# ru1ven/KeypointFusion

Measured on NVIDIA B200. Metric: fusion-path RGB-D samples/sec, higher is better.
Workload: dtype bf16

## Files before the change

keypointfusion_b200/csrc/token_stack.cu:

```cuda
#include "tcgen05.cuh"

namespace kpf {

constexpr int TS_C = 128;
constexpr int TS_WORKERS = 512;
constexpr int TS_NT = TS_WORKERS + 32;
constexpr int TS_RING = 4;
constexpr int TS_SLOT = 2048;
constexpr int TS_MAXG = 64;
constexpr int TS_VEC = 10 * TS_C;
constexpr int TS_PLANE = 512;
constexpr uint32_t ACC_Q = 0, ACC_K = 32, ACC_V = 64, ACC_X = 96, ACC_F = 128, ACC_S = 256, ACC_O = 384;
constexpr uint32_t VT_HI = 128, VT_LO = 144;

struct TokParams {
    const float* x;
    const float* y;
    const float* r3d;
    const float* desa;
    const float* jf;
    const uint4* wmat;
    const int4* wseq;
    const float* wvec;
    float* tokens_out;
    float* pred_out;
    float* out_cj;
    float* out_jc;
    int out_jc_stride, out_jc_c0;
    int B, J, D, L, F, pre, cross, Fc, G, fmt;
    const unsigned long long* peer_bases;
    const int* xstep;
    int world, row0, rows_total;
};

constexpr int XCHG_HEADER_FLOATS = 16;

__device__ __forceinline__ float gelu_erf(float x) {
    const float z = fabsf(x) * 0.70710678118654752f;
    const float t = __fdividef(1.f, 1.f + 0.3275911f * z);
    const float poly = ((((1.061405429f * t - 1.453152027f) * t + 1.421413741f) * t - 0.284496736f) * t + 0.254829592f) * t;
    const float erf_abs = 1.f - poly * __expf(-z * z);
    return 0.5f * x * (1.f + copysignf(erf_abs, x));
}

template <int NV>
__device__ __forceinline__ void warp_reduce_scatter(float* v, int lane) {
    int off = 16;
#pragma unroll
    for (int n = NV; n > 1; n >>= 1, off >>= 1) {
        const bool upper = (lane & off) != 0;
#pragma unroll
        for (int i = 0; i < n / 2; ++i) {
            const float send = upper ? v[i] : v[i + n / 2];
            const float recv = __shfl_xor_sync(0xffffffffu, send, off);
            v[i] = (upper ? v[i + n / 2] : v[i]) + recv;
        }
    }
#pragma unroll
    for (; off > 0; off >>= 1) v[0] += __shfl_xor_sync(0xffffffffu, v[0], off);
}

template <int FMT>
__global__ void __launch_bounds__(TS_NT, 1) token_stack_kernel(const TokParams p) {
    extern __shared__ __align__(128) unsigned char ts_smem[];
    uint4* wslot = reinterpret_cast<uint4*>(ts_smem);
    uint4* bufX = wslot + TS_RING * TS_SLOT;
    uint4* bufY = bufX + 2 * TS_PLANE;
    uint4* bufQ = bufY + 2 * TS_PLANE;
    uint4* bufK = bufQ + 2 * TS_PLANE;
    uint4* bufAt = bufK + 2 * TS_PLANE;
    float* sVec = reinterpret_cast<float*>(bufAt + 128);
    float* sRed = sVec + 2 * TS_VEC;
    float* sSum = sRed + 512;
    float* sHead = sSum + 512;
    float* sLead = sHead + 1024;
    __shared__ __align__(8) uint64_t full[TS_RING], empty[TS_RING], vec_full[2], vec_empty[2], bars[4];
    __shared__ uint32_t tmem_slot;

    const int tid = threadIdx.x, lane = tid & 31, w = tid >> 5, q = w & 3, c = (w >> 2) & 3;
    const int f = 32 * q + lane;
    const int J = p.J, C = TS_C, G = p.G;
    constexpr int fmt = FMT;
    const int b = blockIdx.x;
    const int warp_u = warp_index_uniform();
    const bool producer = warp_u == TS_WORKERS / 32;

    pdl_launch_dependents();
    if (warp_u == 0) tmem_alloc(&tmem_slot, 512);
    if (tid == 32) {
        for (int i = 0; i < TS_RING; ++i) {
            mbar_init(&full[i], 1);
            mbar_init(&empty[i], 1);
        }
        for (int i = 0; i < 2; ++i) {
            mbar_init(&vec_full[i], 1);
            mbar_init(&vec_empty[i], 1);
        }
        for (int i = 0; i < 4; ++i) mbar_init(&bars[i], 1);
        fence_mbar_init();
    }
    tc_fence_before();
    __syncthreads();
    tc_fence_after();
    const uint32_t tmem0 = tmem_slot;
    const uint32_t tmem = tmem0 + ((uint32_t)(32 * q) << 16);

    const int D = p.D, shift = p.L > 0 ? D - C : 0;
    const float* vp = p.wvec;
    const float *qpos = nullptr, *kpos = nullptr, *cross_vec = nullptr, *bfu = nullptr, *pos = nullptr, *bemb = nullptr,
                *Wres_lead = nullptr, *Wres_feat = nullptr, *bres = nullptr, *Wcls = nullptr, *bcls = nullptr, *enc_vec = nullptr;
    if (p.cross) {
        qpos = vp;
        kpos = qpos + J * C;
        cross_vec = kpos + J * C;
        vp = cross_vec + TS_VEC;
    }
    if (p.pre) {
        bfu = vp;
        vp += C;
    }
    if (p.L > 0) {
        pos = vp;
        bemb = pos + J * C;
        Wres_lead = bemb + C;
        Wres_feat = Wres_lead + 48;
        bres = Wres_feat + 3 * C;
        Wcls = bres + 4;
        bcls = Wcls + 3 * C;
        enc_vec = bcls + 4;
    }
    const int n_layers = (p.cross ? 1 : 0) + p.L;
    auto layer_vec = [&](int it) { return (p.cross && it == 0) ? cross_vec : enc_vec + (size_t)(it - (p.cross ? 1 : 0)) * TS_VEC; };

    if (producer) {
        if (elect_one()) {
            for (int e = 0; e < G; ++e) {
                const int4 s = __ldg(p.wseq + e);
                if (s.z >= 0) {
                    const int it = s.z;
                    if (it >= 2) mbar_wait(&vec_empty[it & 1], ((it >> 1) - 1) & 1);
                    mbar_expect_tx(&vec_full[it & 1], TS_VEC * 4);
                    tma_bulk_g2s(sVec + (it & 1) * TS_VEC, layer_vec(it), TS_VEC * 4, &vec_full[it & 1]);
                }
                const int slot = e & (TS_RING - 1);
                if (e >= TS_RING) mbar_wait(&empty[slot], ((e >> 2) - 1) & 1);
                mbar_expect_tx(&full[slot], (uint32_t)s.y * 16);
                tma_bulk_g2s(wslot + slot * TS_SLOT, p.wmat + s.x, (uint32_t)s.y * 16, &full[slot]);
            }
        }
        __syncwarp();
        pdl_wait();
        return;
    }

    auto wsync = [&]() { named_bar_sync(1, 512); };
    uint32_t bar_phase[4] = {0, 0, 0, 0};
    auto wait_bar = [&](int i) {
        mbar_wait(&bars[i], bar_phase[i]);
        bar_phase[i] ^= 1;
        tc_fence_after();
    };
    auto sync_for_mma = [&]() {
        fence_proxy_async();
        tc_fence_before();
        wsync();
    };
    int g = 0;
    auto slot_addr = [&](int e) { return smem_u32(wslot + (e & (TS_RING - 1)) * TS_SLOT); };
    auto wait_full = [&](int e) { mbar_wait(&full[e & (TS_RING - 1)], (e >> 2) & 1); };
    auto issue_proj = [&](uint32_t acc, const uint4* act, int e, bool accumulate) {
        const uint32_t id = umma_idesc_f16(128, 32, false, true, fmt, fmt);
#pragma unroll 1
        for (int h = 0; h < 2; ++h) {
            wait_full(e + h);
            tc_fence_after();
            SmemOp a, bo;
            a.hi = slot_addr(e + h); a.lo = a.hi + 16384; a.lbo = 2048; a.sbo = 128;
            bo.hi = smem_u32(act) + h * 4096; bo.lo = bo.hi + TS_PLANE * 16; bo.lbo = 512; bo.sbo = 128;
            umma_gemm3_ss<64>(tmem0 + acc, a, bo, id, accumulate || h > 0);
            umma_commit(&empty[(e + h) & (TS_RING - 1)]);
        }
    };
    const uint32_t xidx = (uint32_t)((f >> 3) * 32 + c * 8 + (f & 7));
    auto write_act = [&](uint4* buf, const float* v) {
        uint4 hi, lo;
        split8<FMT>(v, hi, lo);
        buf[xidx] = hi;
        buf[TS_PLANE + xidx] = lo;
    };
    bool tokv[8];
#pragma unroll
    for (int i = 0; i < 8; ++i) tokv[i] = 8 * c + i < J;
    auto load_tok = [&](const float* base, int ld, float* v) {
#pragma unroll
        for (int i = 0; i < 8; ++i) v[i] = tokv[i] ? __ldg(base + (size_t)(8 * c + i) * ld + f) : 0.f;
    };
    auto head_partial = [&](int part, const float* v, const float* W) {
        float hx[32];
        const float w0 = __ldg(W + f), w1 = __ldg(W + C + f), w2 = __ldg(W + 2 * C + f);
#pragma unroll
        for (int i = 0; i < 8; ++i) {
            hx[3 * i] = v[i] * w0;
            hx[3 * i + 1] = v[i] * w1;
            hx[3 * i + 2] = v[i] * w2;
        }
#pragma unroll
        for (int i = 24; i < 32; ++i) hx[i] = 0.f;
        warp_reduce_scatter<32>(hx, lane);
        sHead[((part * 4 + q) * 4 + c) * 32 + lane] = hx[0];
    };

    if (tid < 128) sLead[tid] = 0.f;
    wsync();
    pdl_wait();
    float resid[8] = {0.f, 0.f, 0.f, 0.f, 0.f, 0.f, 0.f, 0.f};
    const float qscale = rsqrtf((float)(C / 4));
    int red_par = 0;

    if (p.cross) {
        float a[8], e[8];
        load_tok(p.x + (size_t)b * J * C, C, a);
        load_tok(qpos, C, e);
#pragma unroll
        for (int i = 0; i < 8; ++i) {
            resid[i] = a[i];
            e[i] += a[i];
        }
        write_act(bufX, e);
        load_tok(p.y + (size_t)b * J * C, C, a);
        load_tok(kpos, C, e);
#pragma unroll
        for (int i = 0; i < 8; ++i) e[i] += a[i];
        write_act(bufY, e);
    }

    auto fusion_prologue = [&](float* a) {
        float v[8];
        const float* dsrc = p.desa + (size_t)b * 3 * J * C;
        load_tok(dsrc, C, v);
        write_act(bufX, v);
        load_tok(dsrc + (size_t)J * C, C, v);
        write_act(bufY, v);
        load_tok(dsrc + (size_t)2 * J * C, C, v);
        write_act(bufQ, v);
        load_tok(p.jf + (size_t)b * J * C, C, v);
        write_act(bufK, v);
        sync_for_mma();
        if (warp_u == 0) {
            tc_fence_after();
            if (elect_one()) {
                issue_proj(ACC_X, bufX, g, false);
                issue_proj(ACC_X, bufY, g + 2, true);
                issue_proj(ACC_X, bufQ, g + 4, true);
                issue_proj(ACC_X, bufK, g + 6, true);
                umma_commit(&bars[0]);
            }
            __syncwarp();
        }
        g += 8;
        const float bb = __ldg(bfu + f);
        wait_bar(0);
        tmem_ld<8>(tmem + ACC_X + 8 * c, a);
#pragma unroll
        for (int i = 0; i < 8; ++i) a[i] = tokv[i] ? fmaxf(a[i] + bb, 0.f) : 0.f;
    };
    float pre_a[8] = {0.f, 0.f, 0.f, 0.f, 0.f, 0.f, 0.f, 0.f};
    if (p.pre) {
        fusion_prologue(pre_a);
        if (p.L == 0 && p.tokens_out) {
#pragma unroll
            for (int i = 0; i < 8; ++i)
                if (tokv[i]) p.tokens_out[((size_t)b * J + 8 * c + i) * C + f] = pre_a[i];
        }
    }

    for (int it = 0; it < n_layers; ++it) {
        const bool is_cross = p.cross && it == 0;
        if (it == (p.cross ? 1 : 0) && p.L > 0) {
            if (p.pre) {
                head_partial(0, pre_a, Wres_feat);
                write_act(bufX, pre_a);
            }
            if (!p.pre && !p.cross) {
                float v[8];
                load_tok(p.x + (size_t)b * J * D + shift, D, v);
                head_partial(0, v, Wres_feat);
                write_act(bufX, v);
            }
            if (p.cross) head_partial(0, resid, Wres_feat);
            if (shift > 0 && w == 0) {
                const int t = lane;
                const float* lead = p.cross ? p.r3d + ((size_t)b * J + t) * shift : p.x + ((size_t)b * J + t) * D;
                float tl[16];
#pragma unroll
                for (int i = 0; i < 16; ++i) tl[i] = (t < J && i < shift) ? __ldg(lead + i) : 0.f;
#pragma unroll
                for (int k = 0; k < 3; ++k) {
                    float s = 0.f;
#pragma unroll
                    for (int i = 0; i < 16; ++i) s += tl[i] * __ldg(Wres_lead + 16 * k + i);
                    sLead[4 * t + k] = s;
                }
                uint4 hi, lo;
                split8<FMT>(tl, hi, lo);
                bufAt[t] = hi;
                bufAt[64 + t] = lo;
                split8<FMT>(tl + 8, hi, lo);
                bufAt[32 + t] = hi;
                bufAt[96 + t] = lo;
            }
            sync_for_mma();
            if (warp_u == 0) {
                tc_fence_after();
                if (elect_one()) {
                    issue_proj(ACC_X, bufX, g, false);
                    if (shift > 0) {
                        wait_full(g + 2);
                        tc_fence_after();
                        SmemOp a, bo;
                        a.hi = slot_addr(g + 2); a.lo = a.hi + 256 * 16; a.lbo = 2048; a.sbo = 128;
                        bo.hi = smem_u32(bufAt); bo.lo = bo.hi + 64 * 16; bo.lbo = 512; bo.sbo = 128;
                        umma_gemm3_ss<16>(tmem0 + ACC_X, a, bo, umma_idesc_f16(128, 32, false, false, fmt, fmt), true);
                        umma_commit(&empty[(g + 2) & (TS_RING - 1)]);
                    }
                    umma_commit(&bars[0]);
                }
                __syncwarp();
            }
            g += shift > 0 ? 3 : 2;
            float e[8];
            load_tok(pos, C, e);
            const float bb = __ldg(bemb + f);
            wait_bar(0);
            float a[8];
            tmem_ld<8>(tmem + ACC_X + 8 * c, a);
#pragma unroll
            for (int i = 0; i < 8; ++i) resid[i] = a[i] = tokv[i] ? a[i] + bb + e[i] : 0.f;
            write_act(bufX, a);
        }

        const float* sv = sVec + (it & 1) * TS_VEC;
        const uint4* kv_src = is_cross ? bufY : bufX;
        const int F = is_cross ? p.Fc : p.F;
        const int act = is_cross ? 0 : 1;
        const float eps = is_cross ? 1e-5f : 1e-12f;

        sync_for_mma();
        if (warp_u == 0) {
            tc_fence_after();
            if (elect_one()) {
                if (it >= 1) mbar_arrive(&vec_empty[(it - 1) & 1]);
                issue_proj(ACC_K, kv_src, g, false);
                umma_commit(&bars[1]);
                issue_proj(ACC_Q, bufX, g + 2, false);
                umma_commit(&bars[0]);
            }
            __syncwarp();
        }
        mbar_wait(&vec_full[it & 1], (it >> 1) & 1);
        const float bq = sv[f], bk = sv[C + f], bv = sv[2 * C + f], bo_ = sv[3 * C + f], g1 = sv[4 * C + f], be1 = sv[5 * C + f],
                    b2 = sv[7 * C + f], g2 = sv[8 * C + f], be2 = sv[9 * C + f];
        const float* b1 = sv + 6 * C;
        const uint32_t qidx = (uint32_t)((lane >> 3) * 128 + (4 * q + c) * 8 + (lane & 7));
        wait_bar(1);
        {
            float a[8];
            tmem_ld<8>(tmem + ACC_K + 8 * c, a);
#pragma unroll
            for (int i = 0; i < 8; ++i) a[i] = tokv[i] ? a[i] + bk : 0.f;
            uint4 hi, lo;
            split8<FMT>(a, hi, lo);
            bufK[qidx] = hi;
            bufK[TS_PLANE + qidx] = lo;
        }
        wait_bar(0);
        {
            float a[8];
            tmem_ld<8>(tmem + ACC_Q + 8 * c, a);
#pragma unroll
            for (int i = 0; i < 8; ++i) a[i] = tokv[i] ? (a[i] + bq) * qscale : 0.f;
            uint4 hi, lo;
            split8<FMT>(a, hi, lo);
            bufQ[qidx] = hi;
            bufQ[TS_PLANE + qidx] = lo;
        }
        sync_for_mma();
        if (warp_u == 0) {
            tc_fence_after();
            if (elect_one()) {
                SmemOp a, bo;
                a.hi = smem_u32(bufQ); a.lo = a.hi + TS_PLANE * 16; a.lbo = 2048; a.sbo = 128;
                bo.hi = smem_u32(bufK); bo.lo = bo.hi + TS_PLANE * 16; bo.lbo = 2048; bo.sbo = 128;
                umma_gemm3_ss<32>(tmem0 + ACC_S, a, bo, umma_idesc_f16(128, 128, true, true, fmt, fmt), false);
                umma_commit(&bars[0]);
                issue_proj(ACC_V, kv_src, g + 4, false);
                umma_commit(&bars[1]);
            }
            __syncwarp();
        }
        wait_bar(0);
        {
            float sa[32], own[8];
            tmem_ld_nw<32>(tmem + ACC_S + 32 * q, sa);
            tmem_ld_nw<8>(tmem + ACC_S + 32 * q + 8 * c, own);
            tmem_wait_ld();
            float mx = -INFINITY;
#pragma unroll
            for (int i = 0; i < 32; ++i) mx = fmaxf(mx, i < J ? sa[i] : -INFINITY);
            float psum = 0.f;
            const bool qv = lane < J;
#pragma unroll
            for (int i = 0; i < 8; ++i) {
                own[i] = (qv && tokv[i]) ? __expf(own[i] - mx) : 0.f;
                psum += own[i];
            }
            sSum[c * 128 + f] = psum;
            uint4 hi, lo;
            split8<FMT>(own, hi, lo);
            bufQ[c * 128 + f] = hi;
            bufQ[TS_PLANE + c * 128 + f] = lo;
        }
        wait_bar(1);
        {
            float a[8];
            tmem_ld<8>(tmem + ACC_V + 8 * c, a);
#pragma unroll
            for (int i = 0; i < 8; ++i) a[i] = tokv[i] ? a[i] + bv : 0.f;
            uint4 hi, lo;
            split8<FMT>(a, hi, lo);
            tmem_st_nw<4>(tmem + VT_HI + 4 * c, reinterpret_cast<const float*>(&hi));
            tmem_st_nw<4>(tmem + VT_LO + 4 * c, reinterpret_cast<const float*>(&lo));
            tmem_wait_st();
        }
        sync_for_mma();
        if (warp_u == 0) {
            tc_fence_after();
            if (elect_one()) {
                TmemOp a;
                a.hi = tmem0 + VT_HI; a.lo = tmem0 + VT_LO;
                SmemOp bo;
                bo.hi = smem_u32(bufQ); bo.lo = bo.hi + TS_PLANE * 16; bo.lbo = 2048; bo.sbo = 128;
                umma_gemm3_ts<32>(tmem0 + ACC_O, a, bo, umma_idesc_f16(128, 128, false, false, fmt, fmt), false);
                umma_commit(&bars[0]);
            }
            __syncwarp();
        }
        float inv[8];
        {
            float s8[8] = {0.f, 0.f, 0.f, 0.f, 0.f, 0.f, 0.f, 0.f};
#pragma unroll
            for (int k = 0; k < 4; ++k) {
                const float4 u0 = *reinterpret_cast<const float4*>(sSum + k * 128 + 32 * q + 8 * c);
                const float4 u1 = *reinterpret_cast<const float4*>(sSum + k * 128 + 32 * q + 8 * c + 4);
                s8[0] += u0.x; s8[1] += u0.y; s8[2] += u0.z; s8[3] += u0.w;
                s8[4] += u1.x; s8[5] += u1.y; s8[6] += u1.z; s8[7] += u1.w;
            }
#pragma unroll
            for (int i = 0; i < 8; ++i) inv[i] = tokv[i] ? 1.f / s8[i] : 0.f;
        }
        wait_bar(0);
        {
            float a[8];
            tmem_ld<8>(tmem + ACC_O + 32 * q + 8 * c, a);
#pragma unroll
            for (int i = 0; i < 8; ++i) a[i] *= inv[i];
            write_act(bufX, a);
        }
        auto resid_ln = [&](float bias, float gam, float bet) {
            float v[16];
            tmem_ld<8>(tmem + ACC_X + 8 * c, v);
#pragma unroll
            for (int i = 0; i < 8; ++i) {
                v[i] += bias + resid[i];
                resid[i] = v[i];
                v[8 + i] = v[i] * v[i];
            }
            warp_reduce_scatter<16>(v, lane);
            float* red = sRed + red_par * 256;
            red_par ^= 1;
            if ((lane & 1) == 0) red[(c * 4 + q) * 16 + (lane >> 1)] = v[0];
            wsync();
            float st[16];
#pragma unroll
            for (int i = 0; i < 16; ++i) st[i] = 0.f;
#pragma unroll
            for (int k = 0; k < 4; ++k) {
#pragma unroll
                for (int j4 = 0; j4 < 4; ++j4) {
                    const float4 u = *reinterpret_cast<const float4*>(red + (c * 4 + k) * 16 + 4 * j4);
                    st[4 * j4] += u.x; st[4 * j4 + 1] += u.y; st[4 * j4 + 2] += u.z; st[4 * j4 + 3] += u.w;
                }
            }
            float y[8];
#pragma unroll
            for (int i = 0; i < 8; ++i) {
                const float mean = st[i] * (1.f / C);
                const float rstd = rsqrtf(fmaxf(st[8 + i] * (1.f / C) - mean * mean, 0.f) + eps);
                resid[i] = y[i] = tokv[i] ? (resid[i] - mean) * rstd * gam + bet : 0.f;
            }
            write_act(bufX, y);
        };
        sync_for_mma();
        if (warp_u == 0) {
            tc_fence_after();
            if (elect_one()) {
                issue_proj(ACC_X, bufX, g + 6, false);
                umma_commit(&bars[0]);
            }
            __syncwarp();
        }
        wait_bar(0);
        resid_ln(bo_, g1, be1);
        const int nffn = F == 16 ? 1 : 4;
        sync_for_mma();
        if (warp_u == 0) {
            tc_fence_after();
            if (elect_one()) {
                SmemOp a, bo;
                a.hi = smem_u32(bufX); a.lo = a.hi + TS_PLANE * 16; a.lbo = 512; a.sbo = 128;
                if (F == 16) {
                    wait_full(g + 8);
                    tc_fence_after();
                    bo.hi = slot_addr(g + 8); bo.lo = bo.hi + 256 * 16; bo.lbo = 256; bo.sbo = 128;
                    umma_gemm3_ss<128>(tmem0 + ACC_F, a, bo, umma_idesc_f16(128, 16, true, false, fmt, fmt), false);
                } else {
#pragma unroll 1
                    for (int h = 0; h < 2; ++h) {
                        wait_full(g + 8 + h);
                        tc_fence_after();
                        SmemOp ah = a;
                        ah.hi += h * 4096; ah.lo += h * 4096;
                        bo.hi = slot_addr(g + 8 + h); bo.lo = bo.hi + 16384; bo.lbo = 2048; bo.sbo = 128;
                        umma_gemm3_ss<64>(tmem0 + ACC_F, ah, bo, umma_idesc_f16(128, 128, true, false, fmt, fmt), h > 0);
                        umma_commit(&empty[(g + 8 + h) & (TS_RING - 1)]);
                    }
                }
                umma_commit(&bars[0]);
            }
            __syncwarp();
        }
        wait_bar(0);
        if (q == 0) {
            const bool tv = lane < J;
            if (F == 16) {
                float a[4];
                tmem_ld<4>(tmem0 + ACC_F + 4 * c, a);
#pragma unroll
                for (int i = 0; i < 4; ++i) {
                    const float u = a[i] + b1[4 * c + i];
                    a[i] = tv ? (act == 1 ? gelu_erf(u) : fmaxf(u, 0.f)) : 0.f;
                }
                uint2 hi, lo;
                split2<FMT>(a[0], a[1], hi.x, lo.x);
                split2<FMT>(a[2], a[3], hi.y, lo.y);
                reinterpret_cast<uint2*>(bufY + (c >> 1) * 32 + lane)[c & 1] = hi;
                reinterpret_cast<uint2*>(bufY + TS_PLANE + (c >> 1) * 32 + lane)[c & 1] = lo;
            } else {
#pragma unroll 1
                for (int j4 = 0; j4 < 4; ++j4) {
                    float a[8];
                    tmem_ld<8>(tmem0 + ACC_F + 32 * c + 8 * j4, a);
#pragma unroll
                    for (int i = 0; i < 8; ++i) {
                        const float u = a[i] + b1[32 * c + 8 * j4 + i];
                        a[i] = tv ? (act == 1 ? gelu_erf(u) : fmaxf(u, 0.f)) : 0.f;
                    }
                    uint4 hi, lo;
                    split8<FMT>(a, hi, lo);
                    bufY[(4 * c + j4) * 32 + lane] = hi;
                    bufY[TS_PLANE + (4 * c + j4) * 32 + lane] = lo;
                }
            }
        }
        sync_for_mma();
        if (warp_u == 0) {
            tc_fence_after();
            if (elect_one()) {
                SmemOp a, bo;
                bo.hi = smem_u32(bufY); bo.lo = bo.hi + TS_PLANE * 16; bo.lbo = 512; bo.sbo = 128;
                const uint32_t id = umma_idesc_f16(128, 32, false, false, fmt, fmt);
                if (F == 16) {
                    a.hi = slot_addr(g + 8) + 512 * 16; a.lo = a.hi + 256 * 16; a.lbo = 2048; a.sbo = 128;
                    umma_gemm3_ss<16>(tmem0 + ACC_X, a, bo, id, false);
                    umma_commit(&empty[(g + 8) & (TS_RING - 1)]);
                } else {
#pragma unroll 1
                    for (int h = 0; h < 2; ++h) {
                        wait_full(g + 10 + h);
                        tc_fence_after();
                        a.hi = slot_addr(g + 10 + h); a.lo = a.hi + 16384; a.lbo = 2048; a.sbo = 128;
                        SmemOp bh = bo;
                        bh.hi += h * 4096; bh.lo += h * 4096;
                        umma_gemm3_ss<64>(tmem0 + ACC_X, a, bh, id, h > 0);
                        umma_commit(&empty[(g + 10 + h) & (TS_RING - 1)]);
                    }
                }
                umma_commit(&bars[0]);
            }
            __syncwarp();
        }
        wait_bar(0);
        resid_ln(b2, g2, be2);
        g += 8 + nffn;
    }

    if (p.cross && p.L == 0) {
#pragma unroll
        for (int i = 0; i < 8; ++i) {
            const int t = 8 * c + i;
            if (tokv[i]) {
                if (p.out_cj) p.out_cj[((size_t)b * C + f) * J + t] = resid[i];
                if (p.out_jc) p.out_jc[((size_t)b * J + t) * p.out_jc_stride + p.out_jc_c0 + f] = resid[i];
            }
        }
    }
    if (p.L > 0) {
        head_partial(1, resid, Wcls);
        if (p.tokens_out) {
#pragma unroll
            for (int i = 0; i < 8; ++i)
                if (tokv[i]) p.tokens_out[((size_t)b * J + 8 * c + i) * C + f] = resid[i];
        }
        wsync();
        if (tid < 96 && p.pred_out) {
            const int t = tid / 3, k = tid - 3 * t, cc = t >> 3, i = t & 7;
            if (t < J) {
                float o = __ldg(bres + k) + __ldg(bcls + k) + sLead[4 * t + k];
#pragma unroll
                for (int part = 0; part < 2; ++part)
#pragma unroll
                    for (int qq = 0; qq < 4; ++qq) o += sHead[((part * 4 + qq) * 4 + cc) * 32 + 3 * i + k];
                p.pred_out[((size_t)b * J + t) * 3 + k] = o;
                if (p.peer_bases) {
                    const size_t off = XCHG_HEADER_FLOATS + ((size_t)(*p.xstep & 1) * p.rows_total + p.row0 + b) * J * 3 + (size_t)t * 3 + k;
                    for (int r = 0; r < p.world; ++r) reinterpret_cast<float*>(p.peer_bases[r])[off] = o;
                }
            }
        }
        if (p.peer_bases && tid < 96) {
            __threadfence_system();
            named_bar_sync(2, 96);
            if (tid < p.world) asm volatile("red.relaxed.sys.global.add.u32 [%0], 1;" ::"l"(p.peer_bases[tid]) : "memory");
        }
    }
    tc_fence_before();
    wsync();
    if (warp_u == 0) tmem_dealloc(tmem0, 512);
}

constexpr size_t TS_SMEM = (size_t)(TS_RING * TS_SLOT + 8 * TS_PLANE + 128) * 16 + (size_t)(2 * TS_VEC + 512 + 512 + 1024 + 128) * 4;

}

__global__ void exchange_wait_kernel(const unsigned int* arrived, int* xstep, unsigned int per_step, int* inflight, int mode) {
    if (*inflight) {
        const unsigned int expected = ((unsigned int)*xstep + 1u) * per_step;
        const long long t0 = clock64();
        while (true) {
            unsigned int v;
            asm volatile("ld.acquire.sys.global.u32 %0, [%1];" : "=r"(v) : "l"(arrived) : "memory");
            if ((int)(v - expected) >= 0) break;
            if (clock64() - t0 > 8000000000ll) __trap();
        }
        *xstep = *xstep + 1;
    }
    *inflight = mode == 0 ? 1 : 0;
}

extern "C" int kpf_exchange_wait(const void* exchange_buffer, int* xstep, int samples_per_step, int* inflight, int mode, cudaStream_t stream) {
    KPF_REQUIRE(exchange_buffer != nullptr && xstep != nullptr && inflight != nullptr && samples_per_step >= 1 && (mode == 0 || mode == 1));
    exchange_wait_kernel<<<1, 1, 0, stream>>>((const unsigned int*)exchange_buffer, xstep, (unsigned int)samples_per_step, inflight, mode);
    KPF_CHECK_LAUNCH();
    return 0;
}

extern "C" int kpf_token_stack(const float* x, const float* y, const float* r3d, const float* desa, const float* jf, const void* wmat,
                               const void* wseq, const float* wvec, int n_weights, int cross, int pre, int B, int J, int D, int L, int F,
                               int Fc, int fmt, float* tokens_out, float* pred_out, float* out_cj, float* out_jc, int out_jc_stride,
                               int out_jc_c0, const void* peer_bases, const int* xstep, int world, int row0, int rows_total,
                               cudaStream_t stream) {
    using namespace kpf;
    KPF_REQUIRE(B >= 0 && J >= 1 && J <= 32 && L >= 0 && (cross || pre || L > 0));
    KPF_REQUIRE(fmt == FMT_F16 || fmt == FMT_BF16);
    if (B == 0) return 0;
    KPF_REQUIRE(L == 0 || F == 16 || F == 128);
    KPF_REQUIRE(!cross || (y != nullptr && (Fc == 16 || Fc == 128)));
    KPF_REQUIRE(L == 0 || D == TS_C || (D > TS_C && D <= TS_C + 16));
    KPF_REQUIRE(!pre || (desa != nullptr && jf != nullptr && !cross && (L == 0 || D == TS_C)));
    KPF_REQUIRE(!(cross && L > 0) || (r3d != nullptr && D > TS_C));
    KPF_REQUIRE(n_weights <= TS_MAXG);
    const int per_cross = 8 + (Fc == 16 ? 1 : 4), per_layer = 8 + (F == 16 ? 1 : 4);
    KPF_REQUIRE(n_weights == (cross ? per_cross : 0) + (pre ? 8 : 0) + (L > 0 ? 2 + (D > TS_C ? 1 : 0) + per_layer * L : 0));
    KPF_REQUIRE(((uintptr_t)wmat % 16) == 0 && ((uintptr_t)wseq % 16) == 0);
    TokParams p;
    p.x = x; p.y = y; p.r3d = r3d; p.desa = desa; p.jf = jf; p.wmat = (const uint4*)wmat; p.wseq = (const int4*)wseq; p.wvec = wvec;
    p.tokens_out = tokens_out; p.pred_out = pred_out; p.out_cj = out_cj; p.out_jc = out_jc; p.out_jc_stride = out_jc_stride;
    p.out_jc_c0 = out_jc_c0; p.B = B; p.J = J; p.D = D; p.L = L; p.F = F; p.pre = pre; p.cross = cross; p.Fc = Fc; p.G = n_weights; p.fmt = fmt;
    KPF_REQUIRE(peer_bases == nullptr || (xstep != nullptr && world >= 1 && row0 >= 0 && row0 + B <= rows_total && L > 0));
    p.peer_bases = (const unsigned long long*)peer_bases; p.xstep = xstep; p.world = world; p.row0 = row0; p.rows_total = rows_total;
    auto kern = fmt == FMT_F16 ? token_stack_kernel<FMT_F16> : token_stack_kernel<FMT_BF16>;
    cudaError_t e = kpf::set_smem(kern, TS_SMEM);
    if (e != cudaSuccess) return (int)e;
    e = kpf::launch_pdl(kern, dim3(B), dim3(TS_NT), TS_SMEM, stream, p);
    if (e != cudaSuccess) return (int)e;
    KPF_CHECK_LAUNCH();
    return 0;
}
```

Baseline: 138,300.

## Process two batch samples per CTA with N=64 UMMA tiles

Each CTA now handles two samples, doubling the MMA N dimension from 32 to 64 so every weight tile streamed through the TMA ring is reused across two samples, and the grid is halved. Activation buffers, TMEM accumulator columns and reduction scratch are resized, the weight ring shrinks from 4 to 3 slots to fit shared memory, and the Y buffer is folded into K/Q buffers with the fusion prologue split into two MMA phases. This reduces weight traffic per sample but halves the CTA count, which may leave SMs idle at small batch, and lowers ring depth.

```diff
diff --git a/keypointfusion_b200/csrc/token_stack.cu b/keypointfusion_b200/csrc/token_stack.cu
--- a/keypointfusion_b200/csrc/token_stack.cu
+++ b/keypointfusion_b200/csrc/token_stack.cu
@@ -5,13 +5,14 @@
 constexpr int TS_C = 128;
 constexpr int TS_WORKERS = 512;
 constexpr int TS_NT = TS_WORKERS + 32;
-constexpr int TS_RING = 4;
+constexpr int TS_RING = 3;
 constexpr int TS_SLOT = 2048;
 constexpr int TS_MAXG = 64;
 constexpr int TS_VEC = 10 * TS_C;
-constexpr int TS_PLANE = 512;
-constexpr uint32_t ACC_Q = 0, ACC_K = 32, ACC_V = 64, ACC_X = 96, ACC_F = 128, ACC_S = 256, ACC_O = 384;
-constexpr uint32_t VT_HI = 128, VT_LO = 144;
+constexpr int TS_PLANE = 1024;
+constexpr int TS_HPLANE = 512;
+constexpr uint32_t ACC_Q = 0, ACC_K = 64, ACC_V = 128, ACC_X = 192, ACC_S = 256, ACC_F = 256;
+constexpr uint32_t VT = 0;
 
 struct TokParams {
     const float* x;
@@ -65,15 +66,14 @@
     extern __shared__ __align__(128) unsigned char ts_smem[];
     uint4* wslot = reinterpret_cast<uint4*>(ts_smem);
     uint4* bufX = wslot + TS_RING * TS_SLOT;
-    uint4* bufY = bufX + 2 * TS_PLANE;
-    uint4* bufQ = bufY + 2 * TS_PLANE;
+    uint4* bufQ = bufX + 2 * TS_PLANE;
     uint4* bufK = bufQ + 2 * TS_PLANE;
     uint4* bufAt = bufK + 2 * TS_PLANE;
-    float* sVec = reinterpret_cast<float*>(bufAt + 128);
+    float* sVec = reinterpret_cast<float*>(bufAt + 256);
     float* sRed = sVec + 2 * TS_VEC;
-    float* sSum = sRed + 512;
-    float* sHead = sSum + 512;
-    float* sLead = sHead + 1024;
+    float* sSum = sRed + 1024;
+    float* sHead = sSum + 1024;
+    float* sLead = sHead + 2048;
     __shared__ __align__(8) uint64_t full[TS_RING], empty[TS_RING], vec_full[2], vec_empty[2], bars[4];
     __shared__ uint32_t tmem_slot;
 
@@ -81,7 +81,8 @@
     const int f = 32 * q + lane;
     const int J = p.J, C = TS_C, G = p.G;
     constexpr int fmt = FMT;
-    const int b = blockIdx.x;
+    const int b0 = 2 * blockIdx.x;
+    const bool two = b0 + 1 < p.B;
     const int warp_u = warp_index_uniform();
     const bool producer = warp_u == TS_WORKERS / 32;
 
@@ -142,8 +143,8 @@
                     mbar_expect_tx(&vec_full[it & 1], TS_VEC * 4);
                     tma_bulk_g2s(sVec + (it & 1) * TS_VEC, layer_vec(it), TS_VEC * 4, &vec_full[it & 1]);
                 }
-                const int slot = e & (TS_RING - 1);
-                if (e >= TS_RING) mbar_wait(&empty[slot], ((e >> 2) - 1) & 1);
+                const int slot = e % TS_RING;
+                if (e >= TS_RING) mbar_wait(&empty[slot], (e / TS_RING - 1) & 1);
                 mbar_expect_tx(&full[slot], (uint32_t)s.y * 16);
                 tma_bulk_g2s(wslot + slot * TS_SLOT, p.wmat + s.x, (uint32_t)s.y * 16, &full[slot]);
             }
@@ -166,93 +167,116 @@
         wsync();
     };
     int g = 0;
-    auto slot_addr = [&](int e) { return smem_u32(wslot + (e & (TS_RING - 1)) * TS_SLOT); };
-    auto wait_full = [&](int e) { mbar_wait(&full[e & (TS_RING - 1)], (e >> 2) & 1); };
+    auto slot_addr = [&](int e) { return smem_u32(wslot + (e % TS_RING) * TS_SLOT); };
+    auto wait_full = [&](int e) { mbar_wait(&full[e % TS_RING], (e / TS_RING) & 1); };
     auto issue_proj = [&](uint32_t acc, const uint4* act, int e, bool accumulate) {
-        const uint32_t id = umma_idesc_f16(128, 32, false, true, fmt, fmt);
+        const uint32_t id = umma_idesc_f16(128, 64, false, true, fmt, fmt);
 #pragma unroll 1
         for (int h = 0; h < 2; ++h) {
             wait_full(e + h);
             tc_fence_after();
             SmemOp a, bo;
             a.hi = slot_addr(e + h); a.lo = a.hi + 16384; a.lbo = 2048; a.sbo = 128;
-            bo.hi = smem_u32(act) + h * 4096; bo.lo = bo.hi + TS_PLANE * 16; bo.lbo = 512; bo.sbo = 128;
+            bo.hi = smem_u32(act) + h * 8192; bo.lo = bo.hi + TS_PLANE * 16; bo.lbo = 1024; bo.sbo = 128;
             umma_gemm3_ss<64>(tmem0 + acc, a, bo, id, accumulate || h > 0);
-            umma_commit(&empty[(e + h) & (TS_RING - 1)]);
-        }
-    };
-    const uint32_t xidx = (uint32_t)((f >> 3) * 32 + c * 8 + (f & 7));
-    auto write_act = [&](uint4* buf, const float* v) {
+            umma_commit(&empty[(e + h) % TS_RING]);
+        }
+    };
+    const uint32_t xidx = (uint32_t)((f >> 3) * 64 + c * 8 + (f & 7));
+    auto write_half = [&](uint4* buf, const float* v, int s) {
         uint4 hi, lo;
         split8<FMT>(v, hi, lo);
-        buf[xidx] = hi;
-        buf[TS_PLANE + xidx] = lo;
-    };
-    bool tokv[8];
-#pragma unroll
-    for (int i = 0; i < 8; ++i) tokv[i] = 8 * c + i < J;
-    auto load_tok = [&](const float* base, int ld, float* v) {
-#pragma unroll
-        for (int i = 0; i < 8; ++i) v[i] = tokv[i] ? __ldg(base + (size_t)(8 * c + i) * ld + f) : 0.f;
+        buf[xidx + 32 * s] = hi;
+        buf[TS_PLANE + xidx + 32 * s] = lo;
+    };
+    auto write_act = [&](uint4* buf, const float* v) {
+        write_half(buf, v, 0);
+        write_half(buf, v + 8, 1);
+    };
+    auto load_acc = [&](uint32_t col, float* v) {
+        tmem_ld_nw<8>(tmem + col + 8 * c, v);
+        tmem_ld_nw<8>(tmem + col + 32 + 8 * c, v + 8);
+        tmem_wait_ld();
+    };
+    bool tokv[16];
+#pragma unroll
+    for (int i = 0; i < 16; ++i) tokv[i] = 8 * c + (i & 7) < J && (i < 8 || two);
+    auto load_tok = [&](const float* base, size_t bstride, int ld, float* v) {
+#pragma unroll
+        for (int i = 0; i < 16; ++i)
+            v[i] = tokv[i] ? __ldg(base + (size_t)(b0 + (i >> 3)) * bstride + (size_t)(8 * c + (i & 7)) * ld + f) : 0.f;
     };
     auto head_partial = [&](int part, const float* v, const float* W) {
-        float hx[32];
         const float w0 = __ldg(W + f), w1 = __ldg(W + C + f), w2 = __ldg(W + 2 * C + f);
 #pragma unroll
-        for (int i = 0; i < 8; ++i) {
-            hx[3 * i] = v[i] * w0;
-            hx[3 * i + 1] = v[i] * w1;
-            hx[3 * i + 2] = v[i] * w2;
-        }
-#pragma unroll
-        for (int i = 24; i < 32; ++i) hx[i] = 0.f;
-        warp_reduce_scatter<32>(hx, lane);
-        sHead[((part * 4 + q) * 4 + c) * 32 + lane] = hx[0];
-    };
-
-    if (tid < 128) sLead[tid] = 0.f;
+        for (int s = 0; s < 2; ++s) {
+            float hx[32];
+#pragma unroll
+            for (int i = 0; i < 8; ++i) {
+                hx[3 * i] = v[8 * s + i] * w0;
+                hx[3 * i + 1] = v[8 * s + i] * w1;
+                hx[3 * i + 2] = v[8 * s + i] * w2;
+            }
+#pragma unroll
+            for (int i = 24; i < 32; ++i) hx[i] = 0.f;
+            warp_reduce_scatter<32>(hx, lane);
+            sHead[(((s * 2 + part) * 4 + q) * 4 + c) * 32 + lane] = hx[0];
+        }
+    };
+
+    if (tid < 256) sLead[tid] = 0.f;
     wsync();
     pdl_wait();
-    float resid[8] = {0.f, 0.f, 0.f, 0.f, 0.f, 0.f, 0.f, 0.f};
+    float resid[16];
+#pragma unroll
+    for (int i = 0; i < 16; ++i) resid[i] = 0.f;
     const float qscale = rsqrtf((float)(C / 4));
-    int red_par = 0;
 
     if (p.cross) {
-        float a[8], e[8];
-        load_tok(p.x + (size_t)b * J * C, C, a);
-        load_tok(qpos, C, e);
-#pragma unroll
-        for (int i = 0; i < 8; ++i) {
+        float a[16], e[16];
+        load_tok(p.x, (size_t)J * C, C, a);
+        load_tok(qpos, 0, C, e);
+#pragma unroll
+        for (int i = 0; i < 16; ++i) {
             resid[i] = a[i];
             e[i] += a[i];
         }
         write_act(bufX, e);
-        load_tok(p.y + (size_t)b * J * C, C, a);
-        load_tok(kpos, C, e);
-#pragma unroll
-        for (int i = 0; i < 8; ++i) e[i] += a[i];
-        write_act(bufY, e);
+        load_tok(p.y, (size_t)J * C, C, a);
+        load_tok(kpos, 0, C, e);
+#pragma unroll
+        for (int i = 0; i < 16; ++i) e[i] += a[i];
+        write_act(bufK, e);
     }
 
     auto fusion_prologue = [&](float* a) {
-        float v[8];
-        const float* dsrc = p.desa + (size_t)b * 3 * J * C;
-        load_tok(dsrc, C, v);
+        float v[16];
+        const size_t bs = (size_t)3 * J * C;
+        load_tok(p.desa, bs, C, v);
         write_act(bufX, v);
-        load_tok(dsrc + (size_t)J * C, C, v);
-        write_act(bufY, v);
-        load_tok(dsrc + (size_t)2 * J * C, C, v);
+        load_tok(p.desa + (size_t)J * C, bs, C, v);
         write_act(bufQ, v);
-        load_tok(p.jf + (size_t)b * J * C, C, v);
+        load_tok(p.desa + (size_t)2 * J * C, bs, C, v);
         write_act(bufK, v);
         sync_for_mma();
         if (warp_u == 0) {
             tc_fence_after();
             if (elect_one()) {
                 issue_proj(ACC_X, bufX, g, false);
-                issue_proj(ACC_X, bufY, g + 2, true);
-                issue_proj(ACC_X, bufQ, g + 4, true);
-                issue_proj(ACC_X, bufK, g + 6, true);
+                issue_proj(ACC_X, bufQ, g + 2, true);
+                issue_proj(ACC_X, bufK, g + 4, true);
+                umma_commit(&bars[1]);
+            }
+            __syncwarp();
+        }
+        load_tok(p.jf, (size_t)J * C, C, v);
+        wait_bar(1);
+        write_act(bufX, v);
+        sync_for_mma();
+        if (warp_u == 0) {
+            tc_fence_after();
+            if (elect_one()) {
+                issue_proj(ACC_X, bufX, g + 6, true);
                 umma_commit(&bars[0]);
             }
             __syncwarp();
@@ -260,17 +284,19 @@
         g += 8;
         const float bb = __ldg(bfu + f);
         wait_bar(0);
-        tmem_ld<8>(tmem + ACC_X + 8 * c, a);
-#pragma unroll
-        for (int i = 0; i < 8; ++i) a[i] = tokv[i] ? fmaxf(a[i] + bb, 0.f) : 0.f;
-    };
-    float pre_a[8] = {0.f, 0.f, 0.f, 0.f, 0.f, 0.f, 0.f, 0.f};
+        load_acc(ACC_X, a);
+#pragma unroll
+        for (int i = 0; i < 16; ++i) a[i] = tokv[i] ? fmaxf(a[i] + bb, 0.f) : 0.f;
+    };
+    float pre_a[16];
+#pragma unroll
+    for (int i = 0; i < 16; ++i) pre_a[i] = 0.f;
     if (p.pre) {
         fusion_prologue(pre_a);
         if (p.L == 0 && p.tokens_out) {
 #pragma unroll
-            for (int i = 0; i < 8; ++i)
-                if (tokv[i]) p.tokens_out[((size_t)b * J + 8 * c + i) * C + f] = pre_a[i];
+            for (int i = 0; i < 16; ++i)
+                if (tokv[i]) p.tokens_out[((size_t)(b0 + (i >> 3)) * J + 8 * c + (i & 7)) * C + f] = pre_a[i];
         }
     }
 
@@ -282,32 +308,34 @@
                 write_act(bufX, pre_a);
             }
             if (!p.pre && !p.cross) {
-                float v[8];
-                load_tok(p.x + (size_t)b * J * D + shift, D, v);
+                float v[16];
+                load_tok(p.x + shift, (size_t)J * D, D, v);
                 head_partial(0, v, Wres_feat);
                 write_act(bufX, v);
             }
             if (p.cross) head_partial(0, resid, Wres_feat);
-            if (shift > 0 && w == 0) {
-                const int t = lane;
-                const float* lead = p.cross ? p.r3d + ((size_t)b * J + t) * shift : p.x + ((size_t)b * J + t) * D;
+            if (shift > 0 && w < 2) {
+                const int s = w, t = lane, col = 32 * s + t;
+                const bool ok = t < J && (s == 0 || two);
+                const size_t row = (size_t)(b0 + s) * J + t;
+                const float* lead = p.cross ? p.r3d + row * shift : p.x + row * D;
                 float tl[16];
 #pragma unroll
-                for (int i = 0; i < 16; ++i) tl[i] = (t < J && i < shift) ? __ldg(lead + i) : 0.f;
+                for (int i = 0; i < 16; ++i) tl[i] = (ok && i < shift) ? __ldg(lead + i) : 0.f;
 #pragma unroll
                 for (int k = 0; k < 3; ++k) {
-                    float s = 0.f;
-#pragma unroll
-                    for (int i = 0; i < 16; ++i) s += tl[i] * __ldg(Wres_lead + 16 * k + i);
-                    sLead[4 * t + k] = s;
+                    float sacc = 0.f;
+#pragma unroll
+                    for (int i = 0; i < 16; ++i) sacc += tl[i] * __ldg(Wres_lead + 16 * k + i);
+                    sLead[4 * col + k] = sacc;
                 }
                 uint4 hi, lo;
                 split8<FMT>(tl, hi, lo);
-                bufAt[t] = hi;
-                bufAt[64 + t] = lo;
+                bufAt[col] = hi;
+                bufAt[128 + col] = lo;
                 split8<FMT>(tl + 8, hi, lo);
-                bufAt[32 + t] = hi;
-                bufAt[96 + t] = lo;
+                bufAt[64 + col] = hi;
+                bufAt[192 + col] = lo;
             }
             sync_for_mma();
             if (warp_u == 0) {
@@ -319,28 +347,28 @@
                         tc_fence_after();
                         SmemOp a, bo;
                         a.hi = slot_addr(g + 2); a.lo = a.hi + 256 * 16; a.lbo = 2048; a.sbo = 128;
-                        bo.hi = smem_u32(bufAt); bo.lo = bo.hi + 64 * 16; bo.lbo = 512; bo.sbo = 128;
-                        umma_gemm3_ss<16>(tmem0 + ACC_X, a, bo, umma_idesc_f16(128, 32, false, false, fmt, fmt), true);
-                        umma_commit(&empty[(g + 2) & (TS_RING - 1)]);
+                        bo.hi = smem_u32(bufAt); bo.lo = bo.hi + 128 * 16; bo.lbo = 1024; bo.sbo = 128;
+                        umma_gemm3_ss<16>(tmem0 + ACC_X, a, bo, umma_idesc_f16(128, 64, false, false, fmt, fmt), true);
+                        umma_commit(&empty[(g + 2) % TS_RING]);
                     }
                     umma_commit(&bars[0]);
                 }
                 __syncwarp();
             }
             g += shift > 0 ? 3 : 2;
-            float e[8];
-            load_tok(pos, C, e);
+            float e[16];
+            load_tok(pos, 0, C, e);
             const float bb = __ldg(bemb + f);
             wait_bar(0);
-            float a[8];
-            tmem_ld<8>(tmem + ACC_X + 8 * c, a);
-#pragma unroll
-            for (int i = 0; i < 8; ++i) resid[i] = a[i] = tokv[i] ? a[i] + bb + e[i] : 0.f;
+            float a[16];
+            load_acc(ACC_X, a);
+#pragma unroll
+            for (int i = 0; i < 16; ++i) resid[i] = a[i] = tokv[i] ? a[i] + bb + e[i] : 0.f;
             write_act(bufX, a);
         }
 
         const float* sv = sVec + (it & 1) * TS_VEC;
-        const uint4* kv_src = is_cross ? bufY : bufX;
+        const uint4* kv_src = is_cross ? bufK : bufX;
         const int F = is_cross ? p.Fc : p.F;
         const int act = is_cross ? 0 : 1;
         const float eps = is_cross ? 1e-5f : 1e-12f;
@@ -354,55 +382,67 @@
                 umma_commit(&bars[1]);
                 issue_proj(ACC_Q, bufX, g + 2, false);
                 umma_commit(&bars[0]);
+                if (is_cross) {
+                    issue_proj(ACC_V, kv_src, g + 4, false);
+                    umma_commit(&bars[2]);
+                }
             }
             __syncwarp();
         }
         mbar_wait(&vec_full[it & 1], (it >> 1) & 1);
-        const float bq = sv[f], bk = sv[C + f], bv = sv[2 * C + f], bo_ = sv[3 * C + f], g1 = sv[4 * C + f], be1 = sv[5 * C + f],
-                    b2 = sv[7 * C + f], g2 = sv[8 * C + f], be2 = sv[9 * C + f];
         const float* b1 = sv + 6 * C;
         const uint32_t qidx = (uint32_t)((lane >> 3) * 128 + (4 * q + c) * 8 + (lane & 7));
-        wait_bar(1);
-        {
-            float a[8];
-            tmem_ld<8>(tmem + ACC_K + 8 * c, a);
-#pragma unroll
-            for (int i = 0; i < 8; ++i) a[i] = tokv[i] ? a[i] + bk : 0.f;
+        auto write_heads = [&](uint4* buf, const float* a) {
             uint4 hi, lo;
             split8<FMT>(a, hi, lo);
-            bufK[qidx] = hi;
-            bufK[TS_PLANE + qidx] = lo;
+            buf[qidx] = hi;
+            buf[TS_HPLANE + qidx] = lo;
+            split8<FMT>(a + 8, hi, lo);
+            buf[2 * TS_HPLANE + qidx] = hi;
+            buf[3 * TS_HPLANE + qidx] = lo;
+        };
+        wait_bar(1);
+        if (is_cross) wait_bar(2);
+        {
+            float a[16];
+            load_acc(ACC_K, a);
+#pragma unroll
+            for (int i = 0; i < 16; ++i) a[i] = tokv[i] ? a[i] + sv[C + f] : 0.f;
+            write_heads(bufK, a);
         }
         wait_bar(0);
         {
-            float a[8];
-            tmem_ld<8>(tmem + ACC_Q + 8 * c, a);
-#pragma unroll
-            for (int i = 0; i < 8; ++i) a[i] = tokv[i] ? (a[i] + bq) * qscale : 0.f;
-            uint4 hi, lo;
-            split8<FMT>(a, hi, lo);
-            bufQ[qidx] = hi;
-            bufQ[TS_PLANE + qidx] = lo;
+            float a[16];
+            load_acc(ACC_Q, a);
+#pragma unroll
+            for (int i = 0; i < 16; ++i) a[i] = tokv[i] ? (a[i] + sv[f]) * qscale : 0.f;
+            write_heads(bufQ, a);
         }
         sync_for_mma();
         if (warp_u == 0) {
             tc_fence_after();
             if (elect_one()) {
-                SmemOp a, bo;
-                a.hi = smem_u32(bufQ); a.lo = a.hi + TS_PLANE * 16; a.lbo = 2048; a.sbo = 128;
-                bo.hi = smem_u32(bufK); bo.lo = bo.hi + TS_PLANE * 16; bo.lbo = 2048; bo.sbo = 128;
-                umma_gemm3_ss<32>(tmem0 + ACC_S, a, bo, umma_idesc_f16(128, 128, true, true, fmt, fmt), false);
-                umma_commit(&bars[0]);
-                issue_proj(ACC_V, kv_src, g + 4, false);
-                umma_commit(&bars[1]);
+#pragma unroll
+                for (int s = 0; s < 2; ++s) {
+                    SmemOp a, bo;
+                    a.hi = smem_u32(bufQ + s * 2 * TS_HPLANE); a.lo = a.hi + TS_HPLANE * 16; a.lbo = 2048; a.sbo = 128;
+                    bo.hi = smem_u32(bufK + s * 2 * TS_HPLANE); bo.lo = bo.hi + TS_HPLANE * 16; bo.lbo = 2048; bo.sbo = 128;
+                    umma_gemm3_ss<32>(tmem0 + ACC_S + 128 * s, a, bo, umma_idesc_f16(128, 128, true, true, fmt, fmt), false);
+                    umma_commit(&bars[s]);
+                }
+                if (!is_cross) {
+                    issue_proj(ACC_V, kv_src, g + 4, false);
+                    umma_commit(&bars[2]);
+                }
             }
             __syncwarp();
         }
-        wait_bar(0);
-        {
+#pragma unroll
+        for (int s = 0; s < 2; ++s) {
+            wait_bar(s);
             float sa[32], own[8];
-            tmem_ld_nw<32>(tmem + ACC_S + 32 * q, sa);
-            tmem_ld_nw<8>(tmem + ACC_S + 32 * q + 8 * c, own);
+            tmem_ld_nw<32>(tmem + ACC_S + 128 * s + 32 * q, sa);
+            tmem_ld_nw<8>(tmem + ACC_S + 128 * s + 32 * q + 8 * c, own);
             tmem_wait_ld();
             float mx = -INFINITY;
 #pragma unroll
@@ -411,91 +451,94 @@
             const bool qv = lane < J;
 #pragma unroll
             for (int i = 0; i < 8; ++i) {
-                own[i] = (qv && tokv[i]) ? __expf(own[i] - mx) : 0.f;
+                own[i] = (qv && tokv[8 * s + i]) ? __expf(own[i] - mx) : 0.f;
                 psum += own[i];
             }
-            sSum[c * 128 + f] = psum;
+            sSum[(s * 4 + c) * 128 + f] = psum;
             uint4 hi, lo;
             split8<FMT>(own, hi, lo);
-            bufQ[c * 128 + f] = hi;
-            bufQ[TS_PLANE + c * 128 + f] = lo;
-        }
-        wait_bar(1);
+            bufQ[s * 2 * TS_HPLANE + c * 128 + f] = hi;
+            bufQ[s * 2 * TS_HPLANE + TS_HPLANE + c * 128 + f] = lo;
+        }
+        if (!is_cross) wait_bar(2);
         {
-            float a[8];
-            tmem_ld<8>(tmem + ACC_V + 8 * c, a);
-#pragma unroll
-            for (int i = 0; i < 8; ++i) a[i] = tokv[i] ? a[i] + bv : 0.f;
+            float a[16];
+            load_acc(ACC_V, a);
+#pragma unroll
+            for (int i = 0; i < 16; ++i) a[i] = tokv[i] ? a[i] + sv[2 * C + f] : 0.f;
             uint4 hi, lo;
             split8<FMT>(a, hi, lo);
-            tmem_st_nw<4>(tmem + VT_HI + 4 * c, reinterpret_cast<const float*>(&hi));
-            tmem_st_nw<4>(tmem + VT_LO + 4 * c, reinterpret_cast<const float*>(&lo));
+            tmem_st_nw<4>(tmem + VT + 4 * c, reinterpret_cast<const float*>(&hi));
+            tmem_st_nw<4>(tmem + VT + 16 + 4 * c, reinterpret_cast<const float*>(&lo));
+            split8<FMT>(a + 8, hi, lo);
+            tmem_st_nw<4>(tmem + VT + 32 + 4 * c, reinterpret_cast<const float*>(&hi));
+            tmem_st_nw<4>(tmem + VT + 48 + 4 * c, reinterpret_cast<const float*>(&lo));
             tmem_wait_st();
         }
         sync_for_mma();
         if (warp_u == 0) {
             tc_fence_after();
             if (elect_one()) {
-                TmemOp a;
-                a.hi = tmem0 + VT_HI; a.lo = tmem0 + VT_LO;
-                SmemOp bo;
-                bo.hi = smem_u32(bufQ); bo.lo = bo.hi + TS_PLANE * 16; bo.lbo = 2048; bo.sbo = 128;
-                umma_gemm3_ts<32>(tmem0 + ACC_O, a, bo, umma_idesc_f16(128, 128, false, false, fmt, fmt), false);
+#pragma unroll
+                for (int s = 0; s < 2; ++s) {
+                    TmemOp a;
+                    a.hi = tmem0 + VT + 32 * s; a.lo = a.hi + 16;
+                    SmemOp bo;
+                    bo.hi = smem_u32(bufQ + s * 2 * TS_HPLANE); bo.lo = bo.hi + TS_HPLANE * 16; bo.lbo = 2048; bo.sbo = 128;
+                    umma_gemm3_ts<32>(tmem0 + ACC_S + 128 * s, a, bo, umma_idesc_f16(128, 128, false, false, fmt, fmt), false);
+                }
                 umma_commit(&bars[0]);
             }
             __syncwarp();
         }
-        float inv[8];
-        {
-            float s8[8] = {0.f, 0.f, 0.f, 0.f, 0.f, 0.f, 0.f, 0.f};
+        wait_bar(0);
+#pragma unroll
+        for (int s = 0; s < 2; ++s) {
+            float s8[8] = {0.f, 0.f, 0.f, 0.f, 0.f, 0.f, 0.f, 0.f}, a[8];
+            tmem_ld_nw<8>(tmem + ACC_S + 128 * s + 32 * q + 8 * c, a);
 #pragma unroll
             for (int k = 0; k < 4; ++k) {
-                const float4 u0 = *reinterpret_cast<const float4*>(sSum + k * 128 + 32 * q + 8 * c);
-                const float4 u1 = *reinterpret_cast<const float4*>(sSum + k * 128 + 32 * q + 8 * c + 4);
+                const float4 u0 = *reinterpret_cast<const float4*>(sSum + (s * 4 + k) * 128 + 32 * q + 8 * c);
+                const float4 u1 = *reinterpret_cast<const float4*>(sSum + (s * 4 + k) * 128 + 32 * q + 8 * c + 4);
                 s8[0] += u0.x; s8[1] += u0.y; s8[2] += u0.z; s8[3] += u0.w;
                 s8[4] += u1.x; s8[5] += u1.y; s8[6] += u1.z; s8[7] += u1.w;
             }
-#pragma unroll
-            for (int i = 0; i < 8; ++i) inv[i] = tokv[i] ? 1.f / s8[i] : 0.f;
-        }
-        wait_bar(0);
-        {
-            float a[8];
-            tmem_ld<8>(tmem + ACC_O + 32 * q + 8 * c, a);
-#pragma unroll
-            for (int i = 0; i < 8; ++i) a[i] *= inv[i];
-            write_act(bufX, a);
-        }
-        auto resid_ln = [&](float bias, float gam, float bet) {
-            float v[16];
-            tmem_ld<8>(tmem + ACC_X + 8 * c, v);
-#pragma unroll
-            for (int i = 0; i < 8; ++i) {
+            tmem_wait_ld();
+#pragma unroll
+            for (int i = 0; i < 8; ++i) a[i] *= tokv[8 * s + i] ? 1.f / s8[i] : 0.f;
+            write_half(bufX, a, s);
+        }
+        auto resid_ln = [&](const float* vec, int par) {
+            float v[32];
+            load_acc(ACC_X, v);
+            const float bias = vec[f];
+#pragma unroll
+            for (int i = 0; i < 16; ++i) {
                 v[i] += bias + resid[i];
                 resid[i] = v[i];
-                v[8 + i] = v[i] * v[i];
-            }
-            warp_reduce_scatter<16>(v, lane);
-            float* red = sRed + red_par * 256;
-            red_par ^= 1;
-            if ((lane & 1) == 0) red[(c * 4 + q) * 16 + (lane >> 1)] = v[0];
+                v[16 + i] = v[i] * v[i];
+            }
+            warp_reduce_scatter<32>(v, lane);
+            float* red = sRed + par * 512;
+            red[(c * 4 + q) * 32 + lane] = v[0];
             wsync();
-            float st[16];
-#pragma unroll
-            for (int i = 0; i < 16; ++i) st[i] = 0.f;
+            float st[32];
+#pragma unroll
+            for (int i = 0; i < 32; ++i) st[i] = 0.f;
 #pragma unroll
             for (int k = 0; k < 4; ++k) {
 #pragma unroll
-                for (int j4 = 0; j4 < 4; ++j4) {
-                    const float4 u = *reinterpret_cast<const float4*>(red + (c * 4 + k) * 16 + 4 * j4);
+                for (int j4 = 0; j4 < 8; ++j4) {
+                    const float4 u = *reinterpret_cast<const float4*>(red + (c * 4 + k) * 32 + 4 * j4);
                     st[4 * j4] += u.x; st[4 * j4 + 1] += u.y; st[4 * j4 + 2] += u.z; st[4 * j4 + 3] += u.w;
                 }
             }
-            float y[8];
-#pragma unroll
-            for (int i = 0; i < 8; ++i) {
+            const float gam = vec[C + f], bet = vec[2 * C + f];
+            float y[16];
+#pragma unroll
+            for (int i = 0; i < 16; ++i) {
                 const float mean = st[i] * (1.f / C);
-                const float rstd = rsqrtf(fmaxf(st[8 + i] * (1.f / C) - mean * mean, 0.f) + eps);
+                const float rstd = rsqrtf(fmaxf(st[16 + i] * (1.f / C) - mean * mean, 0.f) + eps);
                 resid[i] = y[i] = tokv[i] ? (resid[i] - mean) * rstd * gam + bet : 0.f;
             }
             write_act(bufX, y);
@@ -510,14 +553,14 @@
             __syncwarp();
         }
         wait_bar(0);
-        resid_ln(bo_, g1, be1);
+        resid_ln(sv + 3 * C, 0);
         const int nffn = F == 16 ? 1 : 4;
         sync_for_mma();
         if (warp_u == 0) {
             tc_fence_after();
             if (elect_one()) {
                 SmemOp a, bo;
-                a.hi = smem_u32(bufX); a.lo = a.hi + TS_PLANE * 16; a.lbo = 512; a.sbo = 128;
+                a.hi = smem_u32(bufX); a.lo = a.hi + TS_PLANE * 16; a.lbo = 1024; a.sbo = 128;
                 if (F == 16) {
                     wait_full(g + 8);
                     tc_fence_after();
@@ -529,10 +572,10 @@
                         wait_full(g + 8 + h);
                         tc_fence_after();
                         SmemOp ah = a;
-                        ah.hi += h * 4096; ah.lo += h * 4096;
+                        ah.hi += h * 8192; ah.lo += h * 8192;
                         bo.hi = slot_addr(g + 8 + h); bo.lo = bo.hi + 16384; bo.lbo = 2048; bo.sbo = 128;
                         umma_gemm3_ss<64>(tmem0 + ACC_F, ah, bo, umma_idesc_f16(128, 128, true, false, fmt, fmt), h > 0);
-                        umma_commit(&empty[(g + 8 + h) & (TS_RING - 1)]);
+                        umma_commit(&empty[(g + 8 + h) % TS_RING]);
                     }
                 }
                 umma_commit(&bars[0]);
@@ -540,11 +583,12 @@
             __syncwarp();
         }
         wait_bar(0);
-        if (q == 0) {
-            const bool tv = lane < J;
+        if (q < 2) {
+            const bool tv = lane < J && (q == 0 || two);
+            uint4* hid = bufK + 32 * q + lane;
             if (F == 16) {
                 float a[4];
-                tmem_ld<4>(tmem0 + ACC_F + 4 * c, a);
+                tmem_ld<4>(tmem + ACC_F + 4 * c, a);
 #pragma unroll
                 for (int i = 0; i < 4; ++i) {
                     const float u = a[i] + b1[4 * c + i];
@@ -553,13 +597,13 @@
                 uint2 hi, lo;
                 split2<FMT>(a[0], a[1], hi.x, lo.x);
                 split2<FMT>(a[2], a[3], hi.y, lo.y);
-                reinterpret_cast<uint2*>(bufY + (c >> 1) * 32 + lane)[c & 1] = hi;
-                reinterpret_cast<uint2*>(bufY + TS_PLANE + (c >> 1) * 32 + lane)[c & 1] = lo;
+                reinterpret_cast<uint2*>(hid + (c >> 1) * 64)[c & 1] = hi;
+                reinterpret_cast<uint2*>(hid + TS_PLANE + (c >> 1) * 64)[c & 1] = lo;
             } else {
 #pragma unroll 1
                 for (int j4 = 0; j4 < 4; ++j4) {
                     float a[8];
-                    tmem_ld<8>(tmem0 + ACC_F + 32 * c + 8 * j4, a);
+                    tmem_ld<8>(tmem + ACC_F + 32 * c + 8 * j4, a);
 #pragma unroll
                     for (int i = 0; i < 8; ++i) {
                         const float u = a[i] + b1[32 * c + 8 * j4 + i];
@@ -567,8 +611,8 @@
                     }
                     uint4 hi, lo;
                     split8<FMT>(a, hi, lo);
-                    bufY[(4 * c + j4) * 32 + lane] = hi;
-                    bufY[TS_PLANE + (4 * c + j4) * 32 + lane] = lo;
+                    hid[(4 * c + j4) * 64] = hi;
+                    hid[TS_PLANE + (4 * c + j4) * 64] = lo;
                 }
             }
         }
@@ -577,12 +621,12 @@
             tc_fence_after();
             if (elect_one()) {
                 SmemOp a, bo;
-                bo.hi = smem_u32(bufY); bo.lo = bo.hi + TS_PLANE * 16; bo.lbo = 512; bo.sbo = 128;
-                const uint32_t id = umma_idesc_f16(128, 32, false, false, fmt, fmt);
+                bo.hi = smem_u32(bufK); bo.lo = bo.hi + TS_PLANE * 16; bo.lbo = 1024; bo.sbo = 128;
+                const uint32_t id = umma_idesc_f16(128, 64, false, false, fmt, fmt);
                 if (F == 16) {
                     a.hi = slot_addr(g + 8) + 512 * 16; a.lo = a.hi + 256 * 16; a.lbo = 2048; a.sbo = 128;
                     umma_gemm3_ss<16>(tmem0 + ACC_X, a, bo, id, false);
-                    umma_commit(&empty[(g + 8) & (TS_RING - 1)]);
+                    umma_commit(&empty[(g + 8) % TS_RING]);
                 } else {
 #pragma unroll 1
                     for (int h = 0; h < 2; ++h) {
@@ -590,9 +634,9 @@
                         tc_fence_after();
                         a.hi = slot_addr(g + 10 + h); a.lo = a.hi + 16384; a.lbo = 2048; a.sbo = 128;
                         SmemOp bh = bo;
-                        bh.hi += h * 4096; bh.lo += h * 4096;
+                        bh.hi += h * 8192; bh.lo += h * 8192;
                         umma_gemm3_ss<64>(tmem0 + ACC_X, a, bh, id, h > 0);
-                        umma_commit(&empty[(g + 10 + h) & (TS_RING - 1)]);
+                        umma_commit(&empty[(g + 10 + h) % TS_RING]);
                     }
                 }
                 umma_commit(&bars[0]);
@@ -600,14 +644,14 @@
             __syncwarp();
         }
         wait_bar(0);
-        resid_ln(b2, g2, be2);
+        resid_ln(sv + 7 * C, 1);
         g += 8 + nffn;
     }
 
     if (p.cross && p.L == 0) {
 #pragma unroll
-        for (int i = 0; i < 8; ++i) {
-            const int t = 8 * c + i;
+        for (int i = 0; i < 16; ++i) {
+            const int b = b0 + (i >> 3), t = 8 * c + (i & 7);
             if (tokv[i]) {
                 if (p.out_cj) p.out_cj[((size_t)b * C + f) * J + t] = resid[i];
                 if (p.out_jc) p.out_jc[((size_t)b * J + t) * p.out_jc_stride + p.out_jc_c0 + f] = resid[i];
@@ -618,29 +662,30 @@
         head_partial(1, resid, Wcls);
         if (p.tokens_out) {
 #pragma unroll
-            for (int i = 0; i < 8; ++i)
-                if (tokv[i]) p.tokens_out[((size_t)b * J + 8 * c + i) * C + f] = resid[i];
+            for (int i = 0; i < 16; ++i)
+                if (tokv[i]) p.tokens_out[((size_t)(b0 + (i >> 3)) * J + 8 * c + (i & 7)) * C + f] = resid[i];
         }
         wsync();
-        if (tid < 96 && p.pred_out) {
-            const int t = tid / 3, k = tid - 3 * t, cc = t >> 3, i = t & 7;
-            if (t < J) {
-                float o = __ldg(bres + k) + __ldg(bcls + k) + sLead[4 * t + k];
+        if (tid < 192 && p.pred_out) {
+            const int s = tid >= 96 ? 1 : 0, r = tid - 96 * s, t = r / 3, k = r - 3 * t, cc = t >> 3, i = t & 7;
+            if (t < J && (s == 0 || two)) {
+                float o = __ldg(bres + k) + __ldg(bcls + k) + sLead[4 * (32 * s + t) + k];
 #pragma unroll
                 for (int part = 0; part < 2; ++part)
 #pragma unroll
-                    for (int qq = 0; qq < 4; ++qq) o += sHead[((part * 4 + qq) * 4 + cc) * 32 + 3 * i + k];
-                p.pred_out[((size_t)b * J + t) * 3 + k] = o;
+                    for (int qq = 0; qq < 4; ++qq) o += sHead[(((s * 2 + part) * 4 + qq) * 4 + cc) * 32 + 3 * i + k];
+                p.pred_out[((size_t)(b0 + s) * J + t) * 3 + k] = o;
                 if (p.peer_bases) {
-                    const size_t off = XCHG_HEADER_FLOATS + ((size_t)(*p.xstep & 1) * p.rows_total + p.row0 + b) * J * 3 + (size_t)t * 3 + k;
+                    const size_t off =
+                        XCHG_HEADER_FLOATS + ((size_t)(*p.xstep & 1) * p.rows_total + p.row0 + b0 + s) * J * 3 + (size_t)t * 3 + k;
                     for (int r = 0; r < p.world; ++r) reinterpret_cast<float*>(p.peer_bases[r])[off] = o;
                 }
             }
         }
-        if (p.peer_bases && tid < 96) {
+        if (p.peer_bases && tid < 192) {
             __threadfence_system();
-            named_bar_sync(2, 96);
-            if (tid < p.world) asm volatile("red.relaxed.sys.global.add.u32 [%0], 1;" ::"l"(p.peer_bases[tid]) : "memory");
+            named_bar_sync(2, 192);
+            if (tid < p.world) asm volatile("red.relaxed.sys.global.add.u32 [%0], %1;" ::"l"(p.peer_bases[tid]), "r"(two ? 2u : 1u) : "memory");
         }
     }
     tc_fence_before();
@@ -648,7 +693,8 @@
     if (warp_u == 0) tmem_dealloc(tmem0, 512);
 }
 
-constexpr size_t TS_SMEM = (size_t)(TS_RING * TS_SLOT + 8 * TS_PLANE + 128) * 16 + (size_t)(2 * TS_VEC + 512 + 512 + 1024 + 128) * 4;
+constexpr size_t TS_SMEM = (size_t)(TS_RING * TS_SLOT + 6 * TS_PLANE + 256) * 16 + (size_t)(2 * TS_VEC + 1024 + 1024 + 2048 + 256) * 4;
+static_assert(TS_SMEM <= 227 * 1024 - 256, "token stack: dynamic + static shared memory above the 227 KB a block may use");
 
 }
 
@@ -701,7 +747,7 @@
     auto kern = fmt == FMT_F16 ? token_stack_kernel<FMT_F16> : token_stack_kernel<FMT_BF16>;
     cudaError_t e = kpf::set_smem(kern, TS_SMEM);
     if (e != cudaSuccess) return (int)e;
-    e = kpf::launch_pdl(kern, dim3(B), dim3(TS_NT), TS_SMEM, stream, p);
+    e = kpf::launch_pdl(kern, dim3((B + 1) / 2), dim3(TS_NT), TS_SMEM, stream, p);
     if (e != cudaSuccess) return (int)e;
     KPF_CHECK_LAUNCH();
     return 0;
```

Result: no change. 138,900 (median of 6 runs) (+0.4%).
